# sara-nl/saraGAN

Hardware: AMD Instinct MI355X
Metric: 3D volumes/sec/node (G+D step) at 128x128x32 (higher is better)
Workload: dtype bf16

## Files before the change

saragan_amd/build.py:

```python
import json
import os
import re
import subprocess
import sys

HERE = os.path.dirname(os.path.abspath(__file__))
CSRC = os.path.join(HERE, 'csrc')
LIB = os.path.join(HERE, 'libsaragan_hip.so')
SOURCES = ['conv3d.hip', 'conv3p.hip', 'conv3w.hip', 'wgrad.hip', 'elementwise.hip', 'optim.hip', 'prof.hip', 'small.hip', 'subpix.hip', 'gemm.hip', 'metrics.hip']
HEADERS = ['common.h', 'prof.h', 'conv_args.h', os.path.join('..', '..', 'include', 'saragan_hip.h')]
FLAGS = ['--offload-arch=gfx950', '-O3', '-std=c++17', '-fPIC', '-Wall', '-Wno-unused-function']
FILE_FLAGS = {'conv3d.hip': ['-fno-slp-vectorize', '-save-temps=obj'], 'wgrad.hip': ['-fno-slp-vectorize', '-save-temps=obj'],
              'subpix.hip': ['-fno-slp-vectorize'], 'conv3p.hip': ['-fno-slp-vectorize', '-save-temps=obj'],
              'conv3w.hip': ['-fno-slp-vectorize', '-save-temps=obj'], 'gemm.hip': ['-fno-slp-vectorize']}


def _hipcc():
    c = os.environ.get('HIPCC')
    if c:
        return c
    return '/opt/rocm/bin/hipcc' if os.path.exists('/opt/rocm/bin/hipcc') else 'hipcc'


def device_asm(source):
    path = os.path.join(HERE, 'build', source.replace('.hip', '') + '-hip-amdgcn-amd-amdhsa-gfx950.s')
    if not os.path.exists(path) or needs_build():
        build(force=True, verbose=False)
    return path


def needs_build():
    if not os.path.exists(LIB):
        return True
    t = os.path.getmtime(LIB)
    deps = [os.path.join(CSRC, s) for s in SOURCES + HEADERS] + [os.path.abspath(__file__)]
    return any(os.path.getmtime(d) > t for d in deps)


RESOURCES = os.path.join(HERE, 'build', 'resource_usage.json')
_REMARK = re.compile(r'remark:\s+(?:\S+:\d+:\d+:\s+)?(Function Name|TotalSGPRs|VGPRs|AGPRs|ScratchSize \[bytes/lane\]|Occupancy \[waves/SIMD\]|'
                     r'SGPRs Spill|VGPRs Spill|LDS Size \[bytes/block\]):\s+(\S+)')
_KEYS = {'TotalSGPRs': 'sgprs', 'VGPRs': 'vgprs', 'AGPRs': 'agprs', 'ScratchSize [bytes/lane]': 'scratch_bytes',
         'Occupancy [waves/SIMD]': 'occupancy', 'SGPRs Spill': 'sgpr_spill', 'VGPRs Spill': 'vgpr_spill',
         'LDS Size [bytes/block]': 'static_lds'}


def parse_resource_remarks(text):
    out, cur = {}, None
    for m in _REMARK.finditer(text):
        k, v = m.group(1), m.group(2)
        if k == 'Function Name':
            cur = out.setdefault(v, {})
        elif cur is not None:
            cur[_KEYS[k]] = int(v)
    return out


def build(force=False, verbose=True):
    if not force and not needs_build() and os.path.exists(RESOURCES):
        return LIB
    objs = []
    os.makedirs(os.path.join(HERE, 'build'), exist_ok=True)
    procs = []
    for s in SOURCES:
        o = os.path.join(HERE, 'build', s.replace('.hip', '.o'))
        objs.append(o)
        cmd = [_hipcc()] + FLAGS + FILE_FLAGS.get(s, []) + ['-Rpass-analysis=kernel-resource-usage', '-c', os.path.join(CSRC, s), '-o', o]
        if verbose:
            print(' '.join(cmd), flush=True)
        log = open(o + '.log', 'w+')
        procs.append((s, subprocess.Popen(cmd, stderr=log), log))
    usage = {}
    for s, p, log in procs:
        rc = p.wait()
        log.seek(0)
        text = log.read()
        log.close()
        if rc != 0:
            sys.stderr.write(text)
            raise RuntimeError(f'hipcc failed on {s}')
        rest = [ln for ln in text.splitlines() if 'kernel-resource-usage' not in ln]
        rest = [ln for i, ln in enumerate(rest) if not _is_remark_context(rest, i)]
        if verbose and any('warning' in ln or 'error' in ln for ln in rest):
            sys.stderr.write('\n'.join(rest) + '\n')
        usage[s] = parse_resource_remarks(text)
    for f_ in os.listdir(os.path.join(HERE, 'build')):
        if f_.endswith(('.bc', '.hipi', '.out', '.hipfb', '.resolution.txt', '-unknown-linux-gnu.s')) or \
                f_.endswith('-gfx950.o'):
            os.unlink(os.path.join(HERE, 'build', f_))
    with open(RESOURCES, 'w') as f:
        json.dump(usage, f, indent=1, sort_keys=True)
    cmd = [_hipcc(), '--offload-arch=gfx950', '-shared', '-fPIC', '-o', LIB] + objs
    if verbose:
        print(' '.join(cmd), flush=True)
    subprocess.check_call(cmd)
    return LIB


def _is_remark_context(lines, i):
    s = lines[i].lstrip()
    return bool(re.match(r'^\d+ \|', s)) or s.startswith('| ^') or s == '|' or s.startswith('^')


def resource_usage():
    build(force=not os.path.exists(RESOURCES), verbose=False)
    with open(RESOURCES) as f:
        return json.load(f)


if __name__ == '__main__':
    build(force='--force' in sys.argv)
    print(LIB)
```

saragan_amd/csrc/common.h:

```cpp
#pragma once
#include <hip/hip_runtime.h>
#include <stdint.h>
#include <mutex>
#include "../../include/saragan_hip.h"

typedef __bf16 bf16_t;
typedef float f32x4 __attribute__((ext_vector_type(4)));
typedef float f32x16 __attribute__((ext_vector_type(16)));
typedef __bf16 bf16x8 __attribute__((ext_vector_type(8)));
typedef __bf16 bf16x4 __attribute__((ext_vector_type(4)));
typedef short s16x4 __attribute__((ext_vector_type(4)));
typedef uint32_t u32x4 __attribute__((ext_vector_type(4)));

#define SG_STORE16_GUARD(v) asm volatile("s_nop 1" ::"v"(v))
typedef uint32_t u32x2 __attribute__((ext_vector_type(2)));

#define SG_LAUNCH_CHECK()                          \
  do {                                             \
    hipError_t e__ = hipGetLastError();            \
    if (e__ != hipSuccess) return (int)e__;        \
  } while (0)

static inline hipStream_t sg_st(sg_stream_t s) { return (hipStream_t)s; }

struct sg_config {
  int fwd_lds, fwd_tg;
  int fwd_v1, fwd_no_pw, fwd_no_dense;
  int fwd_no_v3, fwd_no_v3s, fwd_no_v4, fwd_no_v5, fwd_no_ksplit;
  int fwd3p_16;
  int fwd3s_16;
  int fwd_no_3p;
  int fwd3_gx, fwd3_no_lean;
  int fwd4_gx, fwd4_no_lean, fwd4_no_wres;
  int wgrad_v1, wgrad_no_v3, wgrad_no_lean;
  int wgrad_no_w16;
  int wgrad3l_min_cols;
  int wgrad3l_16;
  int wgrad_v1_blocks;
  int dbg_flags;
  int no_small;
  int deterministic;
  int gemm_ks_model;
  int gemm_k333_maxvox;
  int no_gemm;
};
const sg_config& sg_cfg();

bool sg_gemm_conv_eligible(const sg_conv_shape* s, sg_dtype dt);
size_t sg_gemm_conv_workspace(const sg_conv_shape* s, sg_dtype dt);
int sg_gemm_conv_fwd(const void* x, const void* wp, void* y, const sg_conv_shape* s, const float* bias, int act, float slope,
                     const uint32_t* mask_bits, float mask_slope, uint32_t* sign_out, void* workspace, size_t workspace_bytes,
                     hipStream_t st, bool* used);

bool sg_small_eligible(const sg_conv_shape* s);
bool sg_small_wgrad_eligible(const sg_conv_shape* s);
size_t sg_small_tail_bytes(const sg_conv_shape* s);
size_t sg_small_wgrad_workspace(const sg_conv_shape* s);
int sg_small_pack(const float* w, float coef, int flip, void* tail, const sg_conv_shape* s, sg_dtype dt, hipStream_t st);
int sg_small_fwd(const void* x, const void* tail, void* y, const sg_conv_shape* s, const float* bias, int act, float slope,
                 int pixel_norm, float eps, float* pn_scale, const uint32_t* mask_bits, float mask_slope, uint32_t* sign_out,
                 sg_dtype dt, hipStream_t st);
int sg_small_wgrad(const void* x, const void* dy, float* dw, float* dbias, float coef, void* workspace, size_t workspace_bytes,
                   const sg_conv_shape* s, sg_dtype dt, hipStream_t st);

#define SG_ALLOW_160K_LDS(kern)                                                                                  \
  do {                                                                                                           \
    static std::once_flag once__;                                                                                \
    static hipError_t err__ = hipSuccess;                                                                        \
    std::call_once(once__, [&] {                                                                                 \
      err__ = hipFuncSetAttribute((const void*)(kern), hipFuncAttributeMaxDynamicSharedMemorySize, 160 * 1024);  \
    });                                                                                                          \
    if (err__ != hipSuccess) return (int)err__;                                                                  \
  } while (0)
static inline size_t sg_esize(sg_dtype dt) { return dt == SG_BF16 ? 2 : 4; }
static inline bool sg_aligned16(const void* p) { return (((uintptr_t)p) & 15) == 0; }

struct sg_fastdiv {
  uint32_t d, m;
};
static inline __host__ __device__ sg_fastdiv sg_make_fastdiv(uint32_t d) {
  sg_fastdiv f;
  f.d = d;
  f.m = d <= 1 ? 0u : (uint32_t)((0x100000000ull + d - 1) / d);
  return f;
}
__device__ __forceinline__ uint32_t sg_div(uint32_t x, sg_fastdiv f) {
  return f.d <= 1 ? x : __umulhi(x, f.m);
}

template <typename T>
struct sg_traits;
template <>
struct sg_traits<float> {
  static constexpr int CH = 8;
  __device__ static __forceinline__ float to_f(float v) { return v; }
  __device__ static __forceinline__ float from_f(float v) { return v; }
};
template <>
struct sg_traits<bf16_t> {
  static constexpr int CH = 16;
  __device__ static __forceinline__ float to_f(bf16_t v) { return (float)v; }
  __device__ static __forceinline__ bf16_t from_f(float v) { return (bf16_t)v; }
};

template <typename T>
__device__ __forceinline__ f32x16 sg_mfma_chunk(u32x4 a, u32x4 b, f32x16 c);
template <>
__device__ __forceinline__ f32x16 sg_mfma_chunk<bf16_t>(u32x4 a, u32x4 b, f32x16 c) {
  return __builtin_amdgcn_mfma_f32_32x32x16_bf16(__builtin_bit_cast(bf16x8, a), __builtin_bit_cast(bf16x8, b),
                                                 c, 0, 0, 0);
}
__device__ __forceinline__ void sg_mfma_bf16_acc(f32x16& c, u32x4 a, u32x4 b) {
  asm volatile("v_mfma_f32_32x32x16_bf16 %0, %1, %2, %0" : "+v"(c) : "v"(a), "v"(b));
}
template <int N>
__device__ __forceinline__ void sg_mfma_drain(f32x16 (&acc)[N]) {
  static_assert(N == 2, "extend the operand list");
  asm volatile("s_nop 7\n\ts_nop 7\n\ts_nop 3" : "+v"(acc[0]), "+v"(acc[1]));
}
#define SG_WAIT_LGKM(N) __builtin_amdgcn_s_waitcnt(0xC07F | ((N) << 8))
#define SG_KLOOP_BEGIN() asm volatile("; SG_KLOOP_BEGIN\n\ts_waitcnt lgkmcnt(0)")
#define SG_KLOOP_END() asm volatile("; SG_KLOOP_END")
template <>
__device__ __forceinline__ f32x16 sg_mfma_chunk<float>(u32x4 a, u32x4 b, f32x16 c) {
  f32x4 af = __builtin_bit_cast(f32x4, a), bf = __builtin_bit_cast(f32x4, b);
  c = __builtin_amdgcn_mfma_f32_32x32x2f32(af[0], bf[0], c, 0, 0, 0);
  c = __builtin_amdgcn_mfma_f32_32x32x2f32(af[1], bf[1], c, 0, 0, 0);
  c = __builtin_amdgcn_mfma_f32_32x32x2f32(af[2], bf[2], c, 0, 0, 0);
  c = __builtin_amdgcn_mfma_f32_32x32x2f32(af[3], bf[3], c, 0, 0, 0);
  return c;
}

__device__ __forceinline__ uint32_t sg_sign_word(const f32x16& v, int hh) {
  uint32_t b = 0u;
#pragma unroll
  for (int i = 0; i < 16; ++i) b |= (__float_as_uint(v[i]) >> 31) << ((i & 3) + 8 * (i >> 2));
  b <<= 4 * hh;
  return b | (uint32_t)__shfl_xor((int)b, 32);
}

__device__ __forceinline__ void sg_apply_sign_word(f32x16& v, uint32_t word, int hh, float slope) {
  const uint32_t wsh = word >> (4 * hh);
  const float sm1 = slope - 1.f;
#pragma unroll
  for (int i = 0; i < 16; ++i) {
    const int t = ((int)(wsh << (31 - ((i & 3) + 8 * (i >> 2))))) >> 31;
    v[i] += __uint_as_float((uint32_t)t & __float_as_uint(v[i] * sm1));
  }
}

__device__ __forceinline__ float sg_lrelu(float x, float slope) {
  const float t = x * slope;
  float r;
  asm("v_max_f32 %0, %1, %2" : "=v"(r) : "v"(x), "v"(t));
  return r;
}

__device__ __forceinline__ uint32_t sg_pack_bf16(float lo, float hi) {
  typedef float f32x2_ __attribute__((ext_vector_type(2)));
  typedef __bf16 bf16x2_ __attribute__((ext_vector_type(2)));
  const f32x2_ v = {lo, hi};
  return __builtin_bit_cast(uint32_t, __builtin_convertvector(v, bf16x2_));
}

static inline bool sg_is_pow2f(float g) {
  uint32_t u;
  __builtin_memcpy(&u, &g, 4);
  return g > 0.f && (u & 0x007FFFFFu) == 0 && (u >> 23) != 0 && (u >> 23) != 255;
}

__device__ __forceinline__ u32x4 sg_mask_piece_bf16(u32x4 v, uint32_t m, float gain, float slope) {
  const uint32_t fg = __float_as_uint(gain), fs = __float_as_uint(gain * slope);
  u32x4 o;
#pragma unroll
  for (int e = 0; e < 4; ++e) {
    uint32_t t0, t1, f0, f1;
    asm("v_bfe_i32 %0, %1, %2, 1" : "=v"(t0) : "v"(m), "n"(2 * e));
    asm("v_bfe_i32 %0, %1, %2, 1" : "=v"(t1) : "v"(m), "n"(2 * e + 1));
    asm("v_bfi_b32 %0, %1, %2, %3" : "=v"(f0) : "v"(t0), "v"(fs), "v"(fg));
    asm("v_bfi_b32 %0, %1, %2, %3" : "=v"(f1) : "v"(t1), "v"(fs), "v"(fg));
    const float lo = __uint_as_float(v[e] << 16) * __uint_as_float(f0);
    const float hi = __uint_as_float(v[e] & 0xFFFF0000u) * __uint_as_float(f1);
    o[e] = sg_pack_bf16(lo, hi);
  }
  return o;
}

// ... 121 lines not shown
```

saragan_amd/csrc/prof.hip:

```cpp
#include "prof.h"
#include <mutex>
#include <vector>
#include <string.h>
#include <stdlib.h>
#include <atomic>

namespace {
struct Rec { int kind; sg_conv_shape shape; int dtype; hipEvent_t e0, e1; bool ok; const char* name; };
std::mutex g_mu;
bool g_on = false;
bool g_filter = false;
int g_fkind = 0;
sg_conv_shape g_fshape;
std::vector<Rec> g_recs;
const char* kVersion = "saragan_hip 0.4 (gfx950)";
}

bool sg_prof_on() { return g_on; }
thread_local const char* sg_tls_kernel = "";

namespace {
std::atomic<const sg_config*> g_cfg{nullptr};
int env_int(const char* name, int dflt) {
  const char* v = getenv(name);
  return v && *v ? atoi(v) : dflt;
}
const sg_config* read_config() {
  sg_config* c = new sg_config;
  c->fwd_lds = env_int("SG_FWD_LDS", 80 * 1024);
  c->fwd_tg = env_int("SG_FWD_TG", 0);
  c->fwd_v1 = env_int("SG_FWD_V1", 0);
  c->fwd_no_pw = env_int("SG_FWD_NO_PW", 0);
  c->fwd_no_dense = env_int("SG_FWD_NO_DENSE", 0);
  c->fwd_no_v3 = env_int("SG_FWD_NO_V3", 0);
  c->fwd_no_v3s = env_int("SG_FWD_NO_V3S", 0);
  c->wgrad_no_lean = env_int("SG_WGRAD_NO_LEAN", 0);
  c->wgrad_no_w16 = env_int("SG_WGRAD_NO_W16", 0);
  c->wgrad3l_16 = env_int("SG_WGRAD3L_16", 0);
  c->wgrad3l_min_cols = env_int("SG_WGRAD3L_MIN_COLS", 0);
  c->wgrad_v1_blocks = env_int("SG_WGRAD_V1_BLOCKS", 0);
  c->fwd_no_v4 = env_int("SG_FWD_NO_V4", 0);
  c->fwd_no_v5 = env_int("SG_FWD_NO_V5", 0);
  c->fwd_no_ksplit = env_int("SG_FWD_NO_KSPLIT", 0);
  c->fwd_no_3p = env_int("SG_FWD_NO_3P", 0);
  c->fwd3p_16 = env_int("SG_FWD3P_16", 1);
  c->fwd3s_16 = env_int("SG_FWD3S_16", 1);
  c->fwd3_gx = env_int("SG_FWD3_GX", 0);
  c->fwd3_no_lean = env_int("SG_FWD3_NO_LEAN", 0);
  c->fwd4_gx = env_int("SG_FWD4_GX", 0);
  c->fwd4_no_lean = env_int("SG_FWD4_NO_LEAN", 0);
  c->fwd4_no_wres = env_int("SG_FWD4_NO_WRES", 0);
  c->wgrad_v1 = env_int("SG_WGRAD_V1", 0);
  c->wgrad_no_v3 = env_int("SG_WGRAD_NO_V3", 0);
  c->dbg_flags = env_int("SG_DBG_FLAGS", 0);
  c->no_small = env_int("SG_NO_SMALL", 0);
  c->deterministic = env_int("SG_DETERMINISTIC", 0);
  c->no_gemm = env_int("SG_NO_GEMM", 0);
  c->gemm_ks_model = env_int("SG_GEMM_KS_MODEL", 0);
  c->gemm_k333_maxvox = env_int("SG_GEMM_K333_MAXVOX", 8192);
  return c;
}
}

const sg_config& sg_cfg() {
  const sg_config* c = g_cfg.load(std::memory_order_acquire);
  if (c == nullptr) {
    std::lock_guard<std::mutex> lk(g_mu);
    c = g_cfg.load(std::memory_order_acquire);
    if (c == nullptr) {
      c = read_config();
      g_cfg.store(c, std::memory_order_release);
    }
  }
  return *c;
}

extern "C" int sg_config_reload(void) {
  std::lock_guard<std::mutex> lk(g_mu);
  g_cfg.store(read_config(), std::memory_order_release);
  return SG_OK;
}

void sg_prof_begin(int kind, const sg_conv_shape* s, sg_dtype dt, hipStream_t st, int* slot) {
  std::lock_guard<std::mutex> lk(g_mu);
  if (g_filter && (kind != g_fkind || memcmp(s, &g_fshape, sizeof(sg_conv_shape)) != 0)) { *slot = -1; return; }
  Rec r; r.kind = kind; r.shape = *s; r.dtype = (int)dt; r.ok = false; r.name = "";
  if (hipEventCreate(&r.e0) != hipSuccess) { *slot = -1; return; }
  if (hipEventCreate(&r.e1) != hipSuccess) { (void)hipEventDestroy(r.e0); *slot = -1; return; }
  (void)hipEventRecord(r.e0, st);
  g_recs.push_back(r);
  *slot = (int)g_recs.size() - 1;
}

void sg_prof_end(int slot, hipStream_t st) {
  std::lock_guard<std::mutex> lk(g_mu);
  bool ok = slot >= 0;
  int idx = ok ? slot : -1 - slot;
  if (idx < 0 || idx >= (int)g_recs.size()) return;
  (void)hipEventRecord(g_recs[idx].e1, st);
  g_recs[idx].ok = ok;
}

void sg_prof_name(int slot, const char* name) {
  std::lock_guard<std::mutex> lk(g_mu);
  if (slot >= 0 && slot < (int)g_recs.size()) g_recs[slot].name = name;
}

extern "C" const char* sg_version(void) { return kVersion; }

extern "C" const char* sg_error_string(int code) {
  switch (code) {
    case SG_OK: return "ok";
    case SG_EINVAL: return "invalid argument (shape, null pointer or unsupported combination)";
    case SG_EWORKSPACE: return "workspace too small";
    case SG_EALIGN: return "pointer not 16-byte aligned";
    case SG_EUNSUPPORTED: return "no kernel covers this request";
    default: break;
  }
  if (code > 0) return hipGetErrorString((hipError_t)code);
  return "unknown error";
}

extern "C" int sg_prof_enable(int on) {
  std::lock_guard<std::mutex> lk(g_mu);
  g_on = on != 0;
  if (!g_on) {
    for (auto& r : g_recs) { (void)hipEventDestroy(r.e0); (void)hipEventDestroy(r.e1); }
    g_recs.clear();
  }
  return SG_OK;
}

extern "C" int sg_prof_enabled(void) {
  std::lock_guard<std::mutex> lk(g_mu);
  return g_on ? 1 : 0;
}

extern "C" int sg_prof_set_filter(int kind, const sg_conv_shape* s) {
  std::lock_guard<std::mutex> lk(g_mu);
  g_filter = s != nullptr;
  if (s) { g_fkind = kind; g_fshape = *s; }
  return SG_OK;
}

extern "C" int sg_prof_collect(sg_prof_entry* out, int32_t max_entries, int32_t* n_entries) {
  if (!out || !n_entries || max_entries < 0) return SG_EINVAL;
  std::lock_guard<std::mutex> lk(g_mu);
  int n = 0;
  for (auto& r : g_recs) {
    float ms = 0.f;
    bool ok = r.ok && hipEventSynchronize(r.e1) == hipSuccess && hipEventElapsedTime(&ms, r.e0, r.e1) == hipSuccess;
    (void)hipEventDestroy(r.e0); (void)hipEventDestroy(r.e1);
    if (!ok) continue;
    int j = 0;
    for (; j < n; ++j)
      if (out[j].kind == r.kind && out[j].dtype == r.dtype && memcmp(&out[j].shape, &r.shape, sizeof(sg_conv_shape)) == 0 &&
          strncmp(out[j].kernel, r.name ? r.name : "", sizeof(out[j].kernel) - 1) == 0) break;
    if (j == n) {
      if (n >= max_entries) continue;
      out[n].kind = r.kind; out[n].shape = r.shape; out[n].dtype = r.dtype; out[n].launches = 0; out[n].total_ms = 0;
      const sg_conv_shape& s = r.shape;
      out[n].flops_per_launch = 2.0 * s.n * s.d * s.h * s.w * (double)s.cin * s.cout * s.kd * s.kh * s.kw;
      strncpy(out[n].kernel, r.name ? r.name : "", sizeof(out[n].kernel) - 1);
      out[n].kernel[sizeof(out[n].kernel) - 1] = 0;
      ++n;
    }
    out[j].launches += 1;
    out[j].total_ms += ms;
  }
  g_recs.clear();
  *n_entries = n;
  return SG_OK;
}
```

saragan_amd/csrc/subpix.hip:

```cpp
#include "common.h"
#include "prof.h"
#include <type_traits>

struct SubpixArgs {
  const bf16_t* x;
  const char* wp;
  bf16_t* y;
  const float* bias;
  float* pn_scale;
  uint32_t* sign_out;
  float slope, eps;
  int act, pixel_norm;
  int N, d, h, w, cin, cout, nchunk, ntile;
  int TD, TH, TW;
  int nTd, nTh, nTw;
  int HH, HW, hv;
  int64_t class_stride;
};

namespace {
constexpr int kWHalf = 4 * 8 * 1024;
constexpr int kXMax = 4 * 6 * 34 * 32;

template <int A, int AO>
// ... 728 lines not shown
    }
    sg_static_for<NG>::run([&](auto GG) __attribute__((always_inline)) {
      constexpr int g = decltype(GG)::value;
      {
        const int g4 = g + 4;
        const int c4 = g4 < NG ? chunk : nchunk_i;
        load_w(wr[g & 3], c4, g4 % NG);
      }
      load_y_part(nchunk_i, more, GG);
      const char* ws = wbuf + (g & 1) * kDgW;
      constexpr int FD_ = 3;
      u32x4 xf[FD_], wf[FD_][NT];
      auto read_tap = [&](int slot, int tt) __attribute__((always_inline)) {
        const int tap = g * TPG + tt;
        const int td = tap >> 4, th = (tap >> 2) & 3, tw = tap & 3;
        const int off = (((td & 1) * FH + th) * 2 * PW + (tw & 1) * PW) * 32;
        xf[slot] = *reinterpret_cast<const u32x4*>(ybuf + xb[td >> 1][tw >> 1] + off);
#pragma unroll
        for (int nt = 0; nt < NT; ++nt) wf[slot][nt] = *reinterpret_cast<const u32x4*>(ws + ((tt * NT + nt) << 10) + lane * 16);
      };
#pragma unroll
      for (int tt = 0; tt < FD_ - 1 && tt < TPG; ++tt) read_tap(tt, tt);
#pragma unroll
      for (int tt = 0; tt < TPG; ++tt) {
        if (tt + FD_ - 1 < TPG) read_tap((tt + FD_ - 1) % FD_, tt + FD_ - 1);
        __builtin_amdgcn_sched_barrier(0);
#pragma unroll
        for (int nt = 0; nt < NT; ++nt) acc[nt] = sg_mfma_chunk<bf16_t>(wf[tt % FD_][nt], xf[tt % FD_], acc[nt]);
        __builtin_amdgcn_sched_barrier(0);
      }
      store_w(wr[(g + 1) & 3], wbuf + ((g + 1) & 1) * kDgW);
      __syncthreads();
    });
    if (chunk + 1 == nchunk) {
      const int64_t ov = (((int64_t)on0 * a.d + od0 + vd) * a.h + oh0 + vh) * a.w + ow0 + vw;
#pragma unroll
      for (int nt = 0; nt < NT; ++nt) sg_store_tile_row_bf16(a.gx + ov * a.ci + (cpart * NT + nt) * 32, acc[nt], hh, true);
    }
    store_y();
    __syncthreads();
    if (!more) break;
    ti = nti;
    chunk = nchunk_i;
  }
}

struct SubpixDgradPackArgs {
  const float* w;
  char* wp;
  float coef;
  int ci, co, nchunk, ntile;
};

__global__ void upconv_subpixel_dgrad_pack_kernel(SubpixDgradPackArgs a) {
  const int64_t total = (int64_t)a.nchunk * 64 * a.ntile * 64 * 8;
  for (int64_t i = (int64_t)blockIdx.x * blockDim.x + threadIdx.x; i < total; i += (int64_t)gridDim.x * blockDim.x) {
    int64_t qq = i;
    const int e = (int)(qq % 8); qq /= 8;
    const int lane = (int)(qq % 64); qq /= 64;
    const int ntl = (int)(qq % 2); qq /= 2;
    const int tap = (int)(qq % 64); qq /= 64;
    const int chunk = (int)(qq % a.nchunk);
    const int nt = (int)(qq / a.nchunk) * 2 + ntl;
    const int ci = nt * 32 + (lane & 31), co = chunk * 16 + (lane >> 5) * 8 + e;
    float v = 0.f;
    if (ci < a.ci && co < a.co) {
      const int tj[3] = {tap >> 4, (tap >> 2) & 3, tap & 3};
      int lo[3], hi[3];
#pragma unroll
      for (int k = 0; k < 3; ++k) {
        lo[k] = tj[k] == 0 ? 2 : (tj[k] == 1 ? 1 : 0);
        hi[k] = tj[k] <= 1 ? 2 : (tj[k] == 2 ? 1 : 0);
      }
      for (int kd = lo[0]; kd <= hi[0]; ++kd)
        for (int kh = lo[1]; kh <= hi[1]; ++kh)
          for (int kw = lo[2]; kw <= hi[2]; ++kw)
            v += a.w[((((int64_t)kd * 3 + kh) * 3 + kw) * a.ci + ci) * a.co + co];
      v *= a.coef;
    }
    reinterpret_cast<bf16_t*>(a.wp)[i] = (bf16_t)v;
  }
}

extern "C" int sg_upconv3d_subpixel_dgrad_supported(const sg_conv_shape* s, sg_dtype dt) {
  int td, th, tw;
  if (!s || dt != SG_BF16 || s->cin < 32 || s->cout < 16 || s->cin % 32 || s->cout % 16 || !subpix_tile(s, &td, &th, &tw)) return 0;
  const int nt = s->cin / 32;
  if (nt % 2 || !((tw == 32 && td == 2 && th == 4) || (tw == 16 && td == 2 && th == 8))) return 0;
  if ((int64_t)s->d * s->h * s->w * 8 * s->cout * 2 >= (1ll << 31)) return 0;
  return 1;
}

extern "C" size_t sg_upconv3d_subpixel_dgrad_packed_bytes(const sg_conv_shape* s, sg_dtype dt) {
  if (!s || dt != SG_BF16 || s->cin < 1 || s->cout < 1) return 0;
  return (size_t)sg_cdiv(s->cout, 16) * 64 * sg_cdiv(s->cin, 32) * 1024;
}

extern "C" int sg_upconv3d_subpixel_dgrad_pack(const float* w_dhwio, float coef, void* wp, const sg_conv_shape* s, sg_dtype dt,
                                               sg_stream_t st) {
  if (!s || !w_dhwio || !wp || dt != SG_BF16) return SG_EINVAL;
  SubpixDgradPackArgs a;
  a.w = w_dhwio; a.wp = reinterpret_cast<char*>(wp); a.coef = coef; a.ci = s->cin; a.co = s->cout;
  a.nchunk = sg_cdiv(s->cout, 16); a.ntile = sg_cdiv(s->cin, 32);
  const int64_t total = (int64_t)a.nchunk * 64 * a.ntile * 512;
  int blocks = (int)((total + 255) / 256);
  if (blocks > 4096) blocks = 4096;
  hipLaunchKernelGGL(upconv_subpixel_dgrad_pack_kernel, dim3(blocks), dim3(256), 0, sg_st(st), a);
  SG_LAUNCH_CHECK();
  return SG_OK;
}

extern "C" int sg_upconv3d_subpixel_dgrad(const void* gy, const void* wp, void* gx, const sg_conv_shape* s, sg_dtype dt, sg_stream_t st) {
  if (!s || !gy || !wp || !gx) return SG_EINVAL;
  if (!sg_aligned16(gy) || !sg_aligned16(wp) || !sg_aligned16(gx)) return SG_EALIGN;
  if (!sg_upconv3d_subpixel_dgrad_supported(s, dt)) return SG_EUNSUPPORTED;
  SubpixDgradArgs a;
  int TD, TH, TW;
  subpix_tile(s, &TD, &TH, &TW);
  a.gy = reinterpret_cast<const bf16_t*>(gy); a.wp = reinterpret_cast<const char*>(wp); a.gx = reinterpret_cast<bf16_t*>(gx);
  a.N = s->n; a.d = s->d; a.h = s->h; a.w = s->w; a.ci = s->cin; a.co = s->cout; a.nchunk = s->cout / 16;
  a.nTd = s->d / TD; a.nTh = s->h / TH; a.nTw = s->w / TW;
  a.ntiles = (int64_t)s->n * a.nTd * a.nTh * a.nTw;
  sg_conv_shape full = *s;
  full.d *= 2; full.h *= 2; full.w *= 2; full.kd = full.kh = full.kw = 3; full.upsample_in = 0;
  full.cin = s->cout; full.cout = s->cin;
  sg_prof_scope prof(0, &full, dt, sg_st(st));
  int64_t per_part = 256 / (s->cin / 64) > 8 ? 256 / (s->cin / 64) : 8;
  while (per_part > 8 && per_part > a.ntiles) per_part -= 8;
  const unsigned gx_ = (unsigned)per_part;
  const size_t lds = 2 * (size_t)kDgW + (size_t)kDgY;
  const int nt = s->cin / 32;
  SG_KNAME("upconv_subpixel_dgrad");
#define SG_DG(NT_, TD_, TH_, TW_)                                                    \
  do {                                                                               \
    auto kern = upconv_subpixel_dgrad_kernel<NT_, TD_, TH_, TW_>;                    \
    SG_ALLOW_160K_LDS(kern);                                                         \
    hipLaunchKernelGGL(kern, dim3(gx_, (unsigned)(nt / 2)), dim3(512), lds, sg_st(st), a); \
  } while (0)
  if (TW == 32) SG_DG(2, 2, 4, 32);
  else if (TW == 16) SG_DG(2, 2, 8, 16);
  else { prof.done(SG_EUNSUPPORTED); return SG_EUNSUPPORTED; }
#undef SG_DG
  hipError_t e = hipGetLastError();
  prof.done((int)e);
  return (int)e;
}

struct SubpixWgradArgs {
  const bf16_t* x;
  const bf16_t* gy;
  float* dwt;
  float* dbias;
  int N, d, h, w, cin, cout, ciT, coT;
  int nTh, nTw;
  int64_t ntiles;
  int64_t slab, bslab;
};

namespace {
constexpr int kWX = 3 * 4 * 34 * 64;
constexpr int kWY = 8 * 2 * 32 * 64;
typedef short s16x4_t __attribute__((ext_vector_type(4)));
typedef __attribute__((address_space(3))) s16x4_t* lds_s16x4;

__device__ __forceinline__ bf16x8 sg_tr_frag(const char* p) {
  const s16x4_t lo = __builtin_amdgcn_ds_read_tr16_b64_v4i16((lds_s16x4)p);
  const s16x4_t hi = __builtin_amdgcn_ds_read_tr16_b64_v4i16((lds_s16x4)(p + 256));
  typedef short s16x8_t __attribute__((ext_vector_type(8)));
  const s16x8_t v = {lo[0], lo[1], lo[2], lo[3], hi[0], hi[1], hi[2], hi[3]};
  return __builtin_bit_cast(bf16x8, v);
}
}

__global__ __launch_bounds__(512) void upconv_subpixel_wgrad_kernel(SubpixWgradArgs a) {
  extern __shared__ __attribute__((aligned(16))) char smem[];
  const int tid = threadIdx.x, lane = tid & 63;
  const int cls = __builtin_amdgcn_readfirstlane(tid >> 6);
  const int ca = cls >> 2, cb = (cls >> 1) & 1, cc = cls & 1;
  const int ci_t = blockIdx.y / a.coT, co_t = blockIdx.y % a.coT;
  const bool ones = a.dbias != nullptr && ci_t == 0;
  const int i16 = lane & 15, q16 = lane >> 4;
  const int colb = (16 * (q16 & 1) + 4 * (i16 & 3)) * 2;
  const int kb = 8 * (q16 >> 1) + (i16 >> 2);
  const int D2 = 2 * a.d, H2 = 2 * a.h, W2 = 2 * a.w;
  auto tile_of = [&](int64_t t, int& n, int& dd, int& h0, int& w0) {
    w0 = (int)(t % a.nTw) * 32; t /= a.nTw;
    h0 = (int)(t % a.nTh) * 2; t /= a.nTh;
    dd = (int)(t % a.d);
    n = (int)(t / a.d);
  };
  u32x4 sx[4], sy[4];
  auto load_tile = [&](int64_t t) {
    int n, dd, h0, w0;
    tile_of(t, n, dd, h0, w0);
#pragma unroll
    for (int k = 0; k < 4; ++k) {
      const int p = tid + k * 512;
      const int hv = p >> 2, sub = p & 3;
      const int hw_ = hv % 34, hh_ = (hv / 34) & 3, hd_ = hv / 136;
      const int zd = dd + hd_ - 1, zy = h0 + hh_ - 1, zx = w0 + hw_ - 1;
      const bool ok = p < 1632 && zd >= 0 && zd < a.d && zy >= 0 && zy < a.h && zx >= 0 && zx < a.w;
      const int64_t off = ((((int64_t)n * a.d + (ok ? zd : 0)) * a.h + (ok ? zy : 0)) * a.w + (ok ? zx : 0)) * a.cin + ci_t * 32 + sub * 8;
      const u32x4 v = *reinterpret_cast<const u32x4*>(a.x + off);
      sx[k] = ok ? v : u32x4{0u, 0u, 0u, 0u};
    }
#pragma unroll
    for (int k = 0; k < 4; ++k) {
      const int p = tid + k * 512;
      const int fv = p >> 2, sub = p & 3;
      const int fw = fv & 63, fh = (fv >> 6) & 3, fd = fv >> 8;
      const int64_t off = ((((int64_t)n * D2 + 2 * dd + fd) * H2 + 2 * h0 + fh) * W2 + 2 * w0 + fw) * a.cout + co_t * 32 + sub * 8;
      sy[k] = *reinterpret_cast<const u32x4*>(a.gy + off);
    }
  };
  auto store_tile = [&](char* xb, char* yb) {
#pragma unroll
    for (int k = 0; k < 4; ++k) {
      const int p = tid + k * 512;
      if (p < 1632) *reinterpret_cast<u32x4*>(xb + p * 16) = sx[k];
    }
#pragma unroll
    for (int k = 0; k < 4; ++k) {
      const int p = tid + k * 512;
      const int fv = p >> 2, sub = p & 3;
      const int fw = fv & 63, fh = (fv >> 6) & 3, fd = fv >> 8;
      const int pc = fd * 4 + (fh & 1) * 2 + (fw & 1);
      *reinterpret_cast<u32x4*>(yb + (((pc * 2 + (fh >> 1)) * 32 + (fw >> 1)) << 6) + sub * 16) = sy[k];
    }
  };

  f32x16 acc[9];
#pragma unroll
  for (int j = 0; j < 9; ++j)
#pragma unroll
    for (int i = 0; i < 16; ++i) acc[j][i] = 0.f;
  const bf16x8 one8 = __builtin_bit_cast(bf16x8, u32x4{0x3F803F80u, 0x3F803F80u, 0x3F803F80u, 0x3F803F80u});

  int buf = 0;
  int64_t t = blockIdx.x;
  if (t < a.ntiles) {
    load_tile(t);
    store_tile(smem, smem + kWX);
  }
  __syncthreads();
  for (; t < a.ntiles; t += gridDim.x) {
    const int64_t tn = t + gridDim.x;
    if (tn < a.ntiles) load_tile(tn);
    const char* xb = smem + buf * (kWX + kWY);
    const char* yb = xb + kWX;
#pragma unroll
    for (int th = 0; th < 2; ++th)
#pragma unroll
      for (int wh = 0; wh < 2; ++wh) {
        const bf16x8 bf = sg_tr_frag(yb + (((cls * 2 + th) * 32 + 16 * wh + kb) << 6) + colb);
#pragma unroll
        for (int tap = 0; tap < 8; ++tap) {
          const int tz = tap >> 2, ty = (tap >> 1) & 1, tx = tap & 1;
          const bf16x8 af = sg_tr_frag(xb + ((((ca + tz) * 4 + th + cb + ty) * 34 + 16 * wh + kb + cc + tx) << 6) + colb);
          acc[tap] = __builtin_amdgcn_mfma_f32_32x32x16_bf16(af, bf, acc[tap], 0, 0, 0);
        }
        if (ones) acc[8] = __builtin_amdgcn_mfma_f32_32x32x16_bf16(one8, bf, acc[8], 0, 0, 0);
      }
    if (tn < a.ntiles) store_tile(smem + (buf ^ 1) * (kWX + kWY), smem + (buf ^ 1) * (kWX + kWY) + kWX);
    __syncthreads();
    buf ^= 1;
  }
  const int r = lane & 31, hh = lane >> 5;
  const bool slab = a.slab != 0;
  __syncthreads();
  float* red = reinterpret_cast<float*>(smem);
  if (ones && hh == 0) red[cls * 32 + r] = acc[8][0];
  __syncthreads();
  if (ones && tid < 32) {
    float s = 0.f;
#pragma unroll
    for (int w8 = 0; w8 < 8; ++w8) s += red[w8 * 32 + tid];
    float* dst = a.dbias + (int64_t)blockIdx.x * a.bslab + co_t * 32 + tid;
    if (slab) *dst = s;
    else unsafeAtomicAdd(dst, s);
  }
#pragma unroll
  for (int tap = 0; tap < 8; ++tap) {
    float* dst = a.dwt + (int64_t)blockIdx.x * a.slab + (((((int64_t)cls * 8 + tap) * a.ciT + ci_t) * a.coT + co_t) << 10);
#pragma unroll
    for (int i = 0; i < 16; ++i) {
      const int row = (i & 3) + 8 * (i >> 2) + 4 * hh;
      if (slab) dst[row * 32 + r] = acc[tap][i];
      else unsafeAtomicAdd(dst + row * 32 + r, acc[tap][i]);
    }
  }
}

__global__ void upconv_subpixel_wgrad_finalize_kernel(const float* __restrict__ dwt, float* __restrict__ dw, const float* __restrict__ bsl,
                                                      float* __restrict__ db, float coef, int cin, int cout, int ciT, int coT, int nslab,
                                                      int64_t slab, int64_t bslab) {
  const int64_t total = (int64_t)27 * cin * cout;
  const int64_t i = (int64_t)blockIdx.x * blockDim.x + threadIdx.x;
  if (i < total) {
    const int co = (int)(i % cout);
    const int ci = (int)((i / cout) % cin);
    const int k = (int)(i / ((int64_t)cout * cin));
    const int kk[3] = {k / 9, (k / 3) % 3, k % 3};
    float s = 0.f;
    for (int b = 0; b < nslab; ++b) {
      const float* base = dwt + (int64_t)b * slab;
#pragma unroll
      for (int m = 0; m < 8; ++m) {
        int cls = 0, tap = 0;
#pragma unroll
        for (int dmn = 0; dmn < 3; ++dmn) {
          const int par = (m >> (2 - dmn)) & 1;
          const int tp = kk[dmn] == 0 ? 0 : (kk[dmn] == 2 ? 1 : (par == 0 ? 1 : 0));
          cls = cls * 2 + par;
          tap = tap * 2 + tp;
        }
        s += base[(((((int64_t)cls * 8 + tap) * ciT + (ci >> 5)) * coT + (co >> 5)) << 10) + (ci & 31) * 32 + (co & 31)];
      }
    }
    dw[i] = coef * s;
  }
  if (db != nullptr && bsl != nullptr && i < cout) {
    float s = 0.f;
    for (int b = 0; b < nslab; ++b) s += bsl[(int64_t)b * bslab + i];
    db[i] = s;
  }
}

static int subpix_wgrad_blocks(const sg_conv_shape* s) {
  const int pairs = sg_cdiv(s->cin, 32) * sg_cdiv(s->cout, 32);
  int gx = 256 / pairs;
  if (gx < 8) gx = 8;
  return gx;
}

extern "C" int sg_upconv3d_subpixel_wgrad_supported(const sg_conv_shape* s, sg_dtype dt) {
  return (s && dt == SG_BF16 && s->cin % 32 == 0 && s->cout % 32 == 0 && s->w % 32 == 0 && s->h % 2 == 0 && s->d >= 1 &&
          (int64_t)s->n * s->d * s->h * s->w * 8 * s->cout < (1ll << 40)) ? 1 : 0;
}

extern "C" size_t sg_upconv3d_subpixel_wgrad_workspace(const sg_conv_shape* s, sg_dtype dt) {
  if (!sg_upconv3d_subpixel_wgrad_supported(s, dt)) return 0;
  const size_t tile = (size_t)64 * sg_cdiv(s->cin, 32) * sg_cdiv(s->cout, 32) * 4096;
  const size_t bias = ((size_t)sg_cdiv(s->cout, 32) * 128 + 255) & ~(size_t)255;
  const size_t ns = sg_cfg().deterministic ? (size_t)subpix_wgrad_blocks(s) : 1;
  return ns * (tile + bias);
}

extern "C" int sg_upconv3d_subpixel_wgrad(const void* x, const void* gy, float* dw, float* dbias, float coef, void* workspace,
                                          size_t workspace_bytes, const sg_conv_shape* s, sg_dtype dt, sg_stream_t st) {
  if (!s || !x || !gy || !dw || !workspace) return SG_EINVAL;
  if (!sg_upconv3d_subpixel_wgrad_supported(s, dt)) return SG_EUNSUPPORTED;
  if (!sg_aligned16(x) || !sg_aligned16(gy) || !sg_aligned16(workspace)) return SG_EALIGN;
  if (workspace_bytes < sg_upconv3d_subpixel_wgrad_workspace(s, dt)) return SG_EWORKSPACE;
  hipStream_t hs = sg_st(st);
  SubpixWgradArgs a;
  a.x = reinterpret_cast<const bf16_t*>(x); a.gy = reinterpret_cast<const bf16_t*>(gy);
  a.N = s->n; a.d = s->d; a.h = s->h; a.w = s->w; a.cin = s->cin; a.cout = s->cout;
  a.ciT = s->cin / 32; a.coT = s->cout / 32;
  a.nTh = s->h / 2; a.nTw = s->w / 32;
  a.ntiles = (int64_t)s->n * s->d * a.nTh * a.nTw;
  const bool det = sg_cfg().deterministic != 0;
  const int gx = subpix_wgrad_blocks(s);
  const size_t tile = (size_t)64 * a.ciT * a.coT * 4096;
  const size_t bias = ((size_t)a.coT * 128 + 255) & ~(size_t)255;
  const size_t ns = det ? (size_t)gx : 1;
  a.dwt = reinterpret_cast<float*>(workspace);
  float* bias_ws = reinterpret_cast<float*>(reinterpret_cast<char*>(workspace) + ns * tile);
  a.dbias = dbias ? bias_ws : nullptr;
  a.slab = det ? (int64_t)(tile / 4) : 0;
  a.bslab = det ? (int64_t)(bias / 4) : 0;
  if (!det) {
    hipError_t e = hipMemsetAsync(workspace, 0, tile + bias, hs);
    if (e != hipSuccess) return (int)e;
  }
  sg_conv_shape full = *s;
  full.d *= 2; full.h *= 2; full.w *= 2; full.kd = full.kh = full.kw = 3; full.upsample_in = 1;
  sg_prof_scope prof(1, &full, dt, hs);
  auto kern = upconv_subpixel_wgrad_kernel;
  SG_ALLOW_160K_LDS(kern);
  SG_KNAME("upconv_subpixel_wgrad");
  hipLaunchKernelGGL(kern, dim3((unsigned)gx, (unsigned)(a.ciT * a.coT)), dim3(512), 2 * (size_t)(kWX + kWY), hs, a);
  const int64_t total = (int64_t)27 * s->cin * s->cout;
  hipLaunchKernelGGL(upconv_subpixel_wgrad_finalize_kernel, dim3((unsigned)((total + 255) / 256)), dim3(256), 0, hs, a.dwt, dw,
                     dbias ? bias_ws : nullptr, dbias, coef, s->cin, s->cout, a.ciT, a.coT, (int)ns, a.slab, a.bslab);
  hipError_t e2 = hipGetLastError();
  prof.done((int)e2);
  return (int)e2;
}
```

Before: 617.0.

## Add larger-tile subpixel upconv weight-gradient kernel with double-buffered halo staging

Adds a new default weight-gradient kernel for the subpixel upconvolution that processes 2x4x32 input tiles instead of 1x2x32. It double-buffers the input halo in LDS while prefetching the next tile's activations and output gradients in registers, and stages gradient fragments through a per-wave ring for transposed MFMA loads. The larger tile is meant to reuse each staged input halo across more depth/height taps, cutting global reloads and barriers per unit of work. In exchange it uses more LDS and registers per block, and the old kernel stays reachable through an environment flag.

New measurement: 619.4 (median of 4 runs). About the same (+0.4%).

```diff
diff --git a/saragan_amd/build.py b/saragan_amd/build.py
--- a/saragan_amd/build.py
+++ b/saragan_amd/build.py
@@ -11,7 +11,7 @@
 HEADERS = ['common.h', 'prof.h', 'conv_args.h', os.path.join('..', '..', 'include', 'saragan_hip.h')]
 FLAGS = ['--offload-arch=gfx950', '-O3', '-std=c++17', '-fPIC', '-Wall', '-Wno-unused-function']
 FILE_FLAGS = {'conv3d.hip': ['-fno-slp-vectorize', '-save-temps=obj'], 'wgrad.hip': ['-fno-slp-vectorize', '-save-temps=obj'],
-              'subpix.hip': ['-fno-slp-vectorize'], 'conv3p.hip': ['-fno-slp-vectorize', '-save-temps=obj'],
+              'subpix.hip': ['-fno-slp-vectorize', '-save-temps=obj'], 'conv3p.hip': ['-fno-slp-vectorize', '-save-temps=obj'],
               'conv3w.hip': ['-fno-slp-vectorize', '-save-temps=obj'], 'gemm.hip': ['-fno-slp-vectorize']}
 
 
diff --git a/saragan_amd/csrc/common.h b/saragan_amd/csrc/common.h
--- a/saragan_amd/csrc/common.h
+++ b/saragan_amd/csrc/common.h
@@ -33,6 +33,7 @@
   int fwd3_gx, fwd3_no_lean;
   int fwd4_gx, fwd4_no_lean, fwd4_no_wres;
   int wgrad_v1, wgrad_no_v3, wgrad_no_lean;
+  int subpix_wgrad_v1;
   int wgrad_no_w16;
   int wgrad3l_min_cols;
   int wgrad3l_16;
diff --git a/saragan_amd/csrc/prof.hip b/saragan_amd/csrc/prof.hip
--- a/saragan_amd/csrc/prof.hip
+++ b/saragan_amd/csrc/prof.hip
@@ -52,6 +52,7 @@
   c->fwd4_no_wres = env_int("SG_FWD4_NO_WRES", 0);
   c->wgrad_v1 = env_int("SG_WGRAD_V1", 0);
   c->wgrad_no_v3 = env_int("SG_WGRAD_NO_V3", 0);
+  c->subpix_wgrad_v1 = env_int("SG_SUBPIX_WGRAD_V1", 0);
   c->dbg_flags = env_int("SG_DBG_FLAGS", 0);
   c->no_small = env_int("SG_NO_SMALL", 0);
   c->deterministic = env_int("SG_DETERMINISTIC", 0);
diff --git a/saragan_amd/csrc/subpix.hip b/saragan_amd/csrc/subpix.hip
--- a/saragan_amd/csrc/subpix.hip
+++ b/saragan_amd/csrc/subpix.hip
@@ -904,7 +904,7 @@
   float* dwt;
   float* dbias;
   int N, d, h, w, cin, cout, ciT, coT;
-  int nTh, nTw;
+  int nTd, nTh, nTw;
   int64_t ntiles;
   int64_t slab, bslab;
 };
@@ -1043,6 +1043,165 @@
   }
 }
 
+namespace {
+constexpr int kW2X = 4 * 6 * 34 * 64;
+constexpr int kW2G = 4 * 1024;
+constexpr int kW2Pieces = 4 * 6 * 34 * 4;
+}
+
+__global__ __launch_bounds__(512) void upconv_subpixel_wgrad2_kernel(SubpixWgradArgs a) {
+  extern __shared__ __attribute__((aligned(16))) char smem[];
+  const int tid = threadIdx.x, lane = tid & 63;
+  const int cls = __builtin_amdgcn_readfirstlane(tid >> 6);
+  const int ca = cls >> 2, cb = (cls >> 1) & 1, cc = cls & 1;
+  const int ci_t = blockIdx.y / a.coT, co_t = blockIdx.y % a.coT;
+  const bool ones = a.dbias != nullptr && ci_t == 0;
+  const int i16 = lane & 15, q16 = lane >> 4;
+  const int colb = (16 * (q16 & 1) + 4 * (i16 & 3)) * 2;
+  const int kb = 8 * (q16 >> 1) + (i16 >> 2);
+  const int D2 = 2 * a.d, H2 = 2 * a.h, W2 = 2 * a.w;
+  char* gring = smem + 2 * kW2X + cls * kW2G;
+  const int gk = lane >> 2, gsub = lane & 3;
+  auto tile_of = [&](int64_t t, int& n, int& dd, int& h0, int& w0) {
+    w0 = (int)(t % a.nTw) * 32; t /= a.nTw;
+    h0 = (int)(t % a.nTh) * 4; t /= a.nTh;
+    dd = (int)(t % a.nTd) * 2;
+    n = (int)(t / a.nTd);
+  };
+  u32x4 sx[2];
+  auto load_x = [&](int n, int dd, int h0, int w0, int k0, int cnt) {
+#pragma unroll
+    for (int k = 0; k < cnt; ++k) {
+      const int p = tid + (k0 + k) * 512;
+      const int hv = p >> 2, sub = p & 3;
+      const int hw_ = hv % 34, q = hv / 34, hh_ = q % 6, hd_ = q / 6;
+      const int zd = dd + hd_ - 1, zy = h0 + hh_ - 1, zx = w0 + hw_ - 1;
+      const bool ok = p < kW2Pieces && zd >= 0 && zd < a.d && zy >= 0 && zy < a.h && zx >= 0 && zx < a.w;
+      const int64_t off = ((((int64_t)n * a.d + (ok ? zd : 0)) * a.h + (ok ? zy : 0)) * a.w + (ok ? zx : 0)) * a.cin + ci_t * 32 + sub * 8;
+      const u32x4 v = *reinterpret_cast<const u32x4*>(a.x + off);
+      sx[k] = ok ? v : u32x4{0u, 0u, 0u, 0u};
+    }
+  };
+  auto store_x = [&](char* xb, int k0, int cnt) {
+#pragma unroll
+    for (int k = 0; k < cnt; ++k) {
+      const int p = tid + (k0 + k) * 512;
+      if (p < kW2Pieces) *reinterpret_cast<u32x4*>(xb + p * 16) = sx[k];
+    }
+  };
+  auto load_g = [&](int n, int dd, int h0, int w0, int s, int td) -> u32x4 {
+    const int zd = dd + td, zh = h0 + (s & 3);
+    const bool ok = zd < a.d && zh < a.h;
+    const int64_t off = ((((int64_t)n * D2 + 2 * (ok ? zd : 0) + ca) * H2 + 2 * (ok ? zh : 0) + cb) * W2 + 2 * (w0 + 16 * (s >> 2) + gk) + cc) * a.cout +
+                        co_t * 32 + gsub * 8;
+    const u32x4 v = *reinterpret_cast<const u32x4*>(a.gy + off);
+    return ok ? v : u32x4{0u, 0u, 0u, 0u};
+  };
+
+  f32x16 acc[9];
+#pragma unroll
+  for (int j = 0; j < 9; ++j)
+#pragma unroll
+    for (int i = 0; i < 16; ++i) acc[j][i] = 0.f;
+  const bf16x8 one8 = __builtin_bit_cast(bf16x8, u32x4{0x3F803F80u, 0x3F803F80u, 0x3F803F80u, 0x3F803F80u});
+
+  int buf = 0;
+  int64_t t = blockIdx.x;
+  int n = 0, dd = 0, h0 = 0, w0 = 0;
+  u32x4 gq[2][2];
+#pragma unroll
+  for (int j = 0; j < 4; ++j) gq[j >> 1][j & 1] = u32x4{0u, 0u, 0u, 0u};
+  if (t < a.ntiles) {
+    tile_of(t, n, dd, h0, w0);
+#pragma unroll
+    for (int k0 = 0; k0 < 7; k0 += 2) {
+      load_x(n, dd, h0, w0, k0, k0 + 2 > 7 ? 1 : 2);
+      store_x(smem, k0, k0 + 2 > 7 ? 1 : 2);
+    }
+#pragma unroll
+    for (int j = 0; j < 4; ++j) gq[j >> 1][j & 1] = load_g(n, dd, h0, w0, j >> 1, j & 1);
+  }
+  __syncthreads();
+  for (; t < a.ntiles; t += gridDim.x) {
+    const int64_t tn = t + gridDim.x;
+    const bool more = tn < a.ntiles;
+    int nn = 0, ndd = 0, nh0 = 0, nw0 = 0;
+    if (more) tile_of(tn, nn, ndd, nh0, nw0);
+    const char* xb = smem + buf * kW2X;
+    char* xn = smem + (buf ^ 1) * kW2X;
+#pragma unroll
+    for (int wb = 0; wb < 2; ++wb) {
+      bf16x8 g[2][2];
+#pragma unroll
+      for (int r = 0; r < 5; ++r) {
+        const int k0 = wb * 4 + (r >> 1) * 2, kn = k0 + 2 > 7 ? 7 - k0 : 2;
+        if (more && (r == 0 || r == 2)) load_x(nn, ndd, nh0, nw0, k0, kn);
+        if (r < 4) {
+          const int s = wb * 4 + r;
+#pragma unroll
+          for (int td = 0; td < 2; ++td) *reinterpret_cast<u32x4*>(gring + ((r & 1) * 2 + td) * 1024 + lane * 16) = gq[s & 1][td];
+          __builtin_amdgcn_fence(__ATOMIC_RELEASE, "wavefront");
+          __builtin_amdgcn_wave_barrier();
+          __builtin_amdgcn_fence(__ATOMIC_ACQUIRE, "wavefront");
+#pragma unroll
+          for (int td = 0; td < 2; ++td) g[r & 1][td] = sg_tr_frag(gring + ((r & 1) * 2 + td) * 1024 + (kb << 6) + colb);
+#pragma unroll
+          for (int td = 0; td < 2; ++td) {
+            if (s + 2 < 8) gq[s & 1][td] = load_g(n, dd, h0, w0, s + 2, td);
+            else if (more) gq[s & 1][td] = load_g(nn, ndd, nh0, nw0, s + 2 - 8, td);
+          }
+          if (ones) {
+#pragma unroll
+            for (int td = 0; td < 2; ++td) acc[8] = __builtin_amdgcn_mfma_f32_32x32x16_bf16(one8, g[r & 1][td], acc[8], 0, 0, 0);
+          }
+        }
+#pragma unroll
+        for (int pz = 0; pz < 3; ++pz)
+#pragma unroll
+          for (int tx = 0; tx < 2; ++tx) {
+            const bf16x8 af = sg_tr_frag(xb + ((((ca + pz) * 6 + cb + r) * 34 + 16 * wb + kb + cc + tx) << 6) + colb);
+#pragma unroll
+            for (int tz = 0; tz < 2; ++tz)
+#pragma unroll
+              for (int ty = 0; ty < 2; ++ty) {
+                const int td = pz - tz, th = r - ty;
+                if (td < 0 || td > 1 || th < 0 || th > 3) continue;
+                acc[tz * 4 + ty * 2 + tx] = __builtin_amdgcn_mfma_f32_32x32x16_bf16(af, g[th & 1][td], acc[tz * 4 + ty * 2 + tx], 0, 0, 0);
+              }
+          }
+        if (more && (r == 1 || r == 3)) store_x(xn, k0, kn);
+      }
+    }
+    __syncthreads();
+    buf ^= 1;
+    n = nn; dd = ndd; h0 = nh0; w0 = nw0;
+  }
+  const int r = lane & 31, hh = lane >> 5;
+  const bool slab = a.slab != 0;
+  __syncthreads();
+  float* red = reinterpret_cast<float*>(smem);
+  if (ones && hh == 0) red[cls * 32 + r] = acc[8][0];
+  __syncthreads();
+  if (ones && tid < 32) {
+    float s = 0.f;
+#pragma unroll
+    for (int w8 = 0; w8 < 8; ++w8) s += red[w8 * 32 + tid];
+    float* dst = a.dbias + (int64_t)blockIdx.x * a.bslab + co_t * 32 + tid;
+    if (slab) *dst = s;
+    else unsafeAtomicAdd(dst, s);
+  }
+#pragma unroll
+  for (int tap = 0; tap < 8; ++tap) {
+    float* dst = a.dwt + (int64_t)blockIdx.x * a.slab + (((((int64_t)cls * 8 + tap) * a.ciT + ci_t) * a.coT + co_t) << 10);
+#pragma unroll
+    for (int i = 0; i < 16; ++i) {
+      const int row = (i & 3) + 8 * (i >> 2) + 4 * hh;
+      if (slab) dst[row * 32 + r] = acc[tap][i];
+      else unsafeAtomicAdd(dst + row * 32 + r, acc[tap][i]);
+    }
+  }
+}
+
 __global__ void upconv_subpixel_wgrad_finalize_kernel(const float* __restrict__ dwt, float* __restrict__ dw, const float* __restrict__ bsl,
                                                       float* __restrict__ db, float coef, int cin, int cout, int ciT, int coT, int nslab,
                                                       int64_t slab, int64_t bslab) {
@@ -1109,8 +1268,9 @@
   a.x = reinterpret_cast<const bf16_t*>(x); a.gy = reinterpret_cast<const bf16_t*>(gy);
   a.N = s->n; a.d = s->d; a.h = s->h; a.w = s->w; a.cin = s->cin; a.cout = s->cout;
   a.ciT = s->cin / 32; a.coT = s->cout / 32;
-  a.nTh = s->h / 2; a.nTw = s->w / 32;
-  a.ntiles = (int64_t)s->n * s->d * a.nTh * a.nTw;
+  const bool v1 = sg_cfg().subpix_wgrad_v1 != 0;
+  a.nTd = v1 ? s->d : sg_cdiv(s->d, 2); a.nTh = v1 ? s->h / 2 : sg_cdiv(s->h, 4); a.nTw = s->w / 32;
+  a.ntiles = (int64_t)s->n * a.nTd * a.nTh * a.nTw;
   const bool det = sg_cfg().deterministic != 0;
   const int gx = subpix_wgrad_blocks(s);
   const size_t tile = (size_t)64 * a.ciT * a.coT * 4096;
@@ -1128,10 +1288,18 @@
   sg_conv_shape full = *s;
   full.d *= 2; full.h *= 2; full.w *= 2; full.kd = full.kh = full.kw = 3; full.upsample_in = 1;
   sg_prof_scope prof(1, &full, dt, hs);
-  auto kern = upconv_subpixel_wgrad_kernel;
-  SG_ALLOW_160K_LDS(kern);
-  SG_KNAME("upconv_subpixel_wgrad");
-  hipLaunchKernelGGL(kern, dim3((unsigned)gx, (unsigned)(a.ciT * a.coT)), dim3(512), 2 * (size_t)(kWX + kWY), hs, a);
+  const dim3 grid((unsigned)gx, (unsigned)(a.ciT * a.coT));
+  if (v1) {
+    auto kern = upconv_subpixel_wgrad_kernel;
+    SG_ALLOW_160K_LDS(kern);
+    SG_KNAME("upconv_subpixel_wgrad<v1>");
+    hipLaunchKernelGGL(kern, grid, dim3(512), 2 * (size_t)(kWX + kWY), hs, a);
+  } else {
+    auto kern = upconv_subpixel_wgrad2_kernel;
+    SG_ALLOW_160K_LDS(kern);
+    SG_KNAME("upconv_subpixel_wgrad");
+    hipLaunchKernelGGL(kern, grid, dim3(512), 2 * (size_t)kW2X + 8 * (size_t)kW2G, hs, a);
+  }
   const int64_t total = (int64_t)27 * s->cin * s->cout;
   hipLaunchKernelGGL(upconv_subpixel_wgrad_finalize_kernel, dim3((unsigned)((total + 255) / 256)), dim3(256), 0, hs, a.dwt, dw,
                      dbias ? bias_ws : nullptr, dbias, coef, s->cin, s->cout, a.ciT, a.coT, (int)ns, a.slab, a.bslab);
```
